# PSeitz/veloci

Measured on AMD Instinct MI355X. Metric: queries/sec, 3-term AND on 100M-doc index (p50 latency and HBM fraction alongside), higher is better.
Workload: dtype u32 doc ids + f16->f32 scores

## Files before the change

### veloci_amd/csrc/capi.cpp

```cpp
#include <chrono>
#include <thread>
#include <cstdio>
#include <cstdlib>
#include <cstring>

#include "../../include/veloci_amd.h"
#include <functional>
#include <future>

#include <dlfcn.h>
#include <unistd.h>

#include "engine.hpp"
#include "text.hpp"

using namespace vq;
using vqreq::Request;
using vqreq::VelociError;

namespace {
thread_local std::string g_err;

int fail(int code, const std::string& msg) {
    g_err = msg;
// ... 1547 lines not shown
    ~vq_shard_step() {
        pbs.clear();
        if (idx && idx->comm && idx->comm->unmerged == this) idx->comm->unmerged = nullptr;
        if (counted && idx && idx->comm) {
            idx->comm->live -= 1;
            idx->comm->busy[parity] = false;
        }
    }
};
namespace {
void comm_fail(ShardComm& c, const std::string& why) {
    if (!c.failed.empty()) return;
    c.failed = why;
    if (c.nccl) {
        try {
            if (rccl_api().CommAbort) (void)rccl_api().CommAbort(static_cast<ncclComm_t>(c.nccl));
            c.nccl = nullptr;
        } catch (...) {
        }
    }
}
void bounded_wait(const Index& idx, ShardComm& c, hipEvent_t ev) {
    static const long limit_ms = [] {
        const char* e = std::getenv("VQ_STEP_TIMEOUT_MS");
        return e ? std::atol(e) : 120000L;
    }();
    const auto t0 = std::chrono::steady_clock::now();
    for (uint64_t spins = 0;; ++spins) {
        const hipError_t q = hipEventQuery(ev);
        if (q == hipSuccess) return;
        if (q != hipErrorNotReady) {
            comm_fail(c, std::string("the step's stream reported ") + hipGetErrorString(q));
            throw VelociError(VQ_ERR_DEVICE, "sharded step: " + c.failed);
        }
        if (spins < 2000) continue;
        if ((spins & 63u) == 0) {
            if (c.nccl && rccl_api().CommGetAsyncError) {
                int aerr = 0;
                if (rccl_api().CommGetAsyncError(static_cast<ncclComm_t>(c.nccl), &aerr) == 0 && aerr != 0) {
                    comm_fail(c, std::string("RCCL reported ") + (rccl_api().GetErrorString ? rccl_api().GetErrorString(aerr) : "an error") + " while the step was in flight (a rank is gone)");
                    throw VelociError(VQ_ERR_DEVICE, "sharded step: " + c.failed);
                }
            }
            const long waited = long(std::chrono::duration_cast<std::chrono::milliseconds>(std::chrono::steady_clock::now() - t0).count());
            if (limit_ms > 0 && waited > limit_ms) {
                comm_fail(c, "a step did not complete within " + std::to_string(limit_ms) + " ms (VQ_STEP_TIMEOUT_MS): a rank did not join its exchange");
                throw VelociError(VQ_ERR_DEVICE, "sharded step: " + c.failed);
            }
        }
        std::this_thread::sleep_for(std::chrono::microseconds(20));
    }
    (void)idx;
}
void step_queue_merge(vq_shard_step& step) {
    if (step.merge_queued) return;
    step.merge_queued = true;
    const Index& idx = *step.idx;
    ShardComm& c = *idx.comm;
    if (c.unmerged == &step) c.unmerged = nullptr;
    if (step.used) VQ_HIP(hipStreamWaitEvent(idx.fin_stream, c.ev_xchg[step.parity], 0));
    const uint8_t* gathered = static_cast<const uint8_t*>(c.gathered[step.parity].p);
    for (size_t k = 0; k < step.pbs.size(); ++k)
        finish_launch(idx, *step.pbs[k], step.used && step.pbs[k]->nq_dev ? gathered + step.arena_off[k] : nullptr, uint32_t(c.nranks));
    VQ_HIP(hipEventRecord(c.ev_fin[step.parity], idx.fin_stream));
}
}

int vq_shard_step_begin(const vq_index* index, const vq_request* const* requests, size_t n, vq_shard_step** out) {
    return guard([&] {
        if (!index || !out || (n && !requests)) throw VelociError(VQ_ERR_INVALID_ARGUMENT, "vq_shard_step_begin: null argument");
        *out = nullptr;
        const Index& idx = *index->idx;
        if (!idx.comm) {
            auto local = std::make_unique<ShardComm>();
            comm_setup(const_cast<Index&>(idx), std::move(local));
        }
        ShardComm& c = *idx.comm;
        if (!c.failed.empty()) throw VelociError(VQ_ERR_DEVICE, "vq_shard_step_begin: the communicator is down (" + c.failed + "): make it again (vq_comm_init / vq_comm_init_custom) on every rank");
        const bool exchange = c.nccl != nullptr || c.allgather != nullptr;
        static const bool timing = std::getenv("VQ_TIMING") != nullptr;
        const auto tb0 = std::chrono::steady_clock::now();
        VQ_HIP(hipSetDevice(idx.device));
        const std::vector<const Request*> reqs = request_pointers(requests, n);
        if (c.unmerged) {
            vq_shard_step& prev = *static_cast<vq_shard_step*>(c.unmerged);
            step_queue_merge(prev);
            VQ_HIP(hipStreamWaitEvent(idx.stream, c.ev_fin[prev.parity], 0));
        }
        const auto tb1 = std::chrono::steady_clock::now();
        if (c.live >= 2) throw VelociError(VQ_ERR_INVALID_ARGUMENT, "vq_shard_step_begin: two steps are in flight already (end one first)");
        auto step = std::make_unique<vq_shard_step>();
        step->idx = &idx;
        step->counted = true;
        c.live += 1;
        step->n = n;
        step->parity = c.busy[0] ? 1 : 0;
        if (c.busy[step->parity]) {
            step->counted = false;
            c.live -= 1;
            throw VelociError(VQ_ERR_INVALID_ARGUMENT, "vq_shard_step_begin: both step slots are held (end a step first)");
        }
        c.busy[step->parity] = true;
        auto tb2 = tb1;
        try {
        const size_t chunks_env = [] {
            const char* e = std::getenv("VQ_SHARD_CHUNKS");
            return size_t(e ? std::min(2, std::max(1, std::atoi(e))) : 0);
        }();
        const size_t nchunks = chunks_env && n >= 512 ? chunks_env : 1;
        for (size_t k = 0; k < nchunks; ++k) {
            const size_t b = n * k / nchunks, e = n * (k + 1) / nchunks;
            step->first.push_back(b);
            step->pbs.push_back(run_partial(idx, reqs.data() + b, e - b, step->parity * 2 + int(k)));
        }
        tb2 = std::chrono::steady_clock::now();
        size_t off = 0;
        for (auto& pb : step->pbs) {
            step->arena_off.push_back(off);
            if (exchange && pb->nq_dev) off += (size_t(pb->layout.off_hist) * size_t(c.nranks) + 255) / 256 * 256;
        }
        step->used = off;
        if (off) {
            VQ_HIP(hipEventRecord(c.ev_scan[step->parity], idx.stream));
            VQ_HIP(hipStreamWaitEvent(c.stream, c.ev_scan[step->parity], 0));
            c.gathered[step->parity].ensure(off);
            uint8_t* gathered = c.gathered[step->parity].as<uint8_t>();
            for (size_t k = 0; k < step->pbs.size(); ++k) {
                PartialBatch& pb = *step->pbs[k];
                if (!pb.nq_dev) continue;
                const size_t bytes = size_t(pb.layout.off_hist);
                if (c.nccl) nccl_check(rccl_api().AllGather(pb.d_partial, gathered + step->arena_off[k], bytes, kNcclUint8, static_cast<ncclComm_t>(c.nccl), c.stream), "ncclAllGather");
                else if (c.allgather(c.ctx, pb.d_partial, gathered + step->arena_off[k], bytes, c.stream) != 0) throw VelociError(VQ_ERR_DEVICE, "sharded step: the caller's all-gather failed");
                if (pb.layout.total_hist) {
                    void* h = pb.d_partial + pb.layout.off_hist;
                    if (c.nccl) nccl_check(rccl_api().AllReduce(h, h, size_t(pb.layout.total_hist), kNcclUint32, kNcclSum, static_cast<ncclComm_t>(c.nccl), c.stream), "ncclAllReduce");
                    else if (!c.allreduce_u32 || c.allreduce_u32(c.ctx, h, size_t(pb.layout.total_hist), c.stream) != 0)
                        throw VelociError(VQ_ERR_DEVICE, "sharded step: the caller's all-reduce failed");
                }
            }
            VQ_HIP(hipEventRecord(c.ev_xchg[step->parity], c.stream));
        }
        } catch (const std::exception& ex) {
            if (exchange && c.nranks > 1) comm_fail(c, std::string("a step failed on rank ") + std::to_string(c.rank) + ": " + ex.what());
            throw;
        }
        c.unmerged = step.get();
        *out = step.release();
        if (timing) {
            const auto tb3 = std::chrono::steady_clock::now();
            auto ms = [](auto a, auto b) { return std::chrono::duration<double, std::milli>(b - a).count(); };
            std::fprintf(stderr, "[vq timing] shard step begin %.3f ms (queue the previous merge %.3f, compile + scans %.3f, exchange calls %.3f)\n", ms(tb0, tb3), ms(tb0, tb1), ms(tb1, tb2), ms(tb2, tb3));
        }
    });
}

int vq_shard_step_end(vq_shard_step* step_raw, size_t stride, uint64_t* num_hits, uint32_t* counts, uint32_t* ids, float* scores, int* status) {
    std::unique_ptr<vq_shard_step> step(step_raw);
    return guard([&] {
        if (!step || (step->n && (!num_hits || !counts || !ids || !scores))) throw VelociError(VQ_ERR_INVALID_ARGUMENT, "vq_shard_step_end: null argument");
        const Index& idx = *step->idx;
        ShardComm& c = *idx.comm;
        VQ_HIP(hipSetDevice(idx.device));
        static const bool timing = std::getenv("VQ_TIMING") != nullptr;
        const auto te0 = std::chrono::steady_clock::now();
        if (!c.failed.empty()) throw VelociError(VQ_ERR_DEVICE, "vq_shard_step_end: the communicator is down (" + c.failed + ")");
        step_queue_merge(*step);
// ... 86 lines not shown
```

### veloci_amd/csrc/engine.hpp

```cpp
#pragma once
#include <hip/hip_runtime.h>

#include <atomic>
#include <cmath>
#include <chrono>
#include <cstdint>
#include <cstdlib>
#include <map>
#include <limits>
#include <memory>
#include <thread>
#include <functional>
#include <condition_variable>
#include <mutex>
#include <string>
#include <unordered_map>
#include <vector>

#include "device_types.hpp"
#include "kernels.hpp"
#include "request.hpp"
#include "hostpool.hpp"
#include "regex_dfa.hpp"

// ... 456 lines not shown
    void* unmerged = nullptr;
    int live = 0;
    DevBuf gathered[2];
    DevBuf red;
    bool busy[2] = {false, false};
    std::string failed;
    std::mutex mu;
    ~ShardComm();
};

struct Index {
    int device = 0;
    int (*allreduce_fn)(void*, uint64_t*, size_t) = nullptr;
    void* allreduce_ctx = nullptr;
    bool sharded() const { return doc_lo != 0 || doc_hi != num_anchors; }
    bool can_sum_over_shards() const { return !sharded() || allreduce_fn != nullptr; }
    void sum_over_shards(std::vector<uint64_t>& v) const {
        if (!sharded() || v.empty()) return;
        if (!allreduce_fn || allreduce_fn(allreduce_ctx, v.data(), v.size()) != 0) throw vqreq::VelociError(vqreq::ERR_DEVICE, "all-reduce over the shards failed");
    }
    struct HighlightField {
        std::once_flag once;
        bool ok = false;
        uint32_t num_texts = 0;
        const KVStore* t2t = nullptr;
        const KVStore* tokens = nullptr;
        const uint32_t* d_vals = nullptr;
        DevBuf own_vals;
    };
    mutable std::mutex highlight_mu;
    mutable std::map<std::string, std::unique_ptr<HighlightField>> highlight_fields;
    mutable std::atomic<uint64_t> highlight_device_parts{0}, highlight_snippets_built{0};
    mutable std::atomic<uint64_t> suggest_topn_probes{0}, suggest_records_back{0};
    mutable std::atomic<uint64_t> or_reruns{0};
    mutable std::unique_ptr<HostPool> pool;
    mutable std::mutex pool_mu;
    uint64_t uid = 0;
    uint32_t num_anchors = 0, doc_lo = 0, doc_hi = 0;
    uint32_t bitmap_base = 0;
    uint64_t bitmap_words = 0;
    std::map<std::string, Dictionary> dict;
    std::map<std::string, PostingStore> postings;
    std::map<std::string, KVStore> kv;
    std::map<std::string, PhraseStore> phrase;
    std::map<std::string, BoostColumn> boost;
    std::map<std::string, ColumnMeta> columns;
    uint64_t device_bytes = 0;
    mutable std::mutex composed_mu;
    mutable std::map<std::string, std::unique_ptr<KVStore>> composed_facets;
    const KVStore& composed_facet(const std::vector<std::string>& steps) const;
    hipStream_t own_stream = nullptr, own_fin_stream = nullptr;
    hipStream_t pre_stream = nullptr;
    hipStream_t stream = nullptr;
    hipStream_t fin_stream = nullptr;
    mutable std::mutex profile_mutex;
    mutable Profile profile;
    mutable Workspace ws[kWorkspaces];
    mutable std::atomic<uint32_t> next_ws{0};
    mutable DevBuf arena;
    static constexpr size_t kArenaBytes = 64ull << 20;
    mutable std::unique_ptr<ShardComm> comm;
    ~Index();
    bool is_anchor_identity(const std::string& textindex_path) const;
};

std::unique_ptr<Index> build_index(const IndexBuilder& b, int device);

struct DocSet {
    uint64_t index_uid = 0;
    uint32_t num_anchors = 0, doc_lo = 0, doc_hi = 0;
    uint64_t len = 0;
    uint32_t local_len = 0;
    uint64_t bitmap_words = 0, rank_entries = 0, tile_entries = 0;
    DevBuf docs, bitmap, rank_dir, tile_dir;
    uint64_t device_bytes = 0;
    float ms_mark = -1.0f, ms_count_scan = -1.0f, ms_expand = -1.0f;
    int route = -1;
    int device = 0;
    hipStream_t stream = nullptr;
};
using DocSetMarkFn = std::function<void(hipStream_t st, uint32_t* scratch, uint64_t scratch_words, unsigned long long* meta)>;
std::shared_ptr<DocSet> docset_from_marks(const Index& idx, hipStream_t st, uint64_t n, const DocSetMarkFn& mark);
inline uint64_t docset_scratch_words(const Index& idx) { return ((uint64_t(idx.num_anchors) + 511u) / 512u) * 16u; }
std::shared_ptr<const DocSet> make_docset(const Index& idx, const uint32_t* ids, uint64_t n, bool on_device);
std::shared_ptr<const DocSet> make_docset_from_program(const Index& idx, hipStream_t st, const DList* lists, uint32_t n_lists, const DOp* fops, uint32_t n_fops,
                                                       uint32_t stack_depth);
enum { SETOP_AND = 0, SETOP_OR = 1, SETOP_MINUS = 2, SETOP_NOT = 3 };
std::shared_ptr<const DocSet> combine_docsets(const Index& idx, int op, const std::vector<std::shared_ptr<const DocSet>>& sets);
uint64_t copy_docset_ids(const DocSet& ds, uint32_t* out, uint64_t cap, bool on_device);

struct HList {
    const uint32_t* d_docs = nullptr;
    const uint16_t* d_scores = nullptr;
    uint32_t len = 0;
    uint32_t flags = 0;
    float term_score = 0.f;
    uint16_t max_raw = 0x7C00;
    uint16_t pivot_raw = 0x7C00;
    float max_value = std::numeric_limits<float>::infinity();
    uint64_t global_len = 0;
    const uint32_t* d_bitmap = nullptr;
    const uint32_t* d_rank_dir = nullptr;
    const uint32_t* d_tile_dir = nullptr;
    const uint32_t* d_cov32 = nullptr;
    const uint16_t* d_arr16 = nullptr;
    const uint32_t* d_gdir = nullptr;
// ... 114 lines not shown
    uint32_t n_spans = 0, tile_words = 0;
    struct Node {
        uint32_t id;
        uint64_t hits, hits_in_filter;
    };
    std::vector<Node> nodes;
};
std::vector<NodeCounts> debug_node_counts(const Index& idx, const vqreq::Request* const* reqs, size_t n, bool summed);
struct Result;
void complete_explain_requests(const Index& idx, std::vector<std::unique_ptr<Result>>& results, std::vector<int>& status, std::vector<std::string>& errors);
void complete_why_found_requests(const Index& idx, std::vector<std::unique_ptr<Result>>& results, std::vector<int>& status, std::vector<std::string>& errors);
bool request_wants_explain(const vqreq::Request& req);
std::string explain_records_json(const ExplainRecs& records);
void complete_deep_requests(const Index& idx, const vqreq::Request* const* reqs, size_t n, std::vector<std::unique_ptr<Result>>& results,
                            std::vector<int>& status, std::vector<std::string>& errors);

struct ResultFacet {
    std::string field;
    std::vector<std::pair<std::string, uint64_t>> entries;
};
struct Result {
    uint64_t num_hits = 0;
    uint64_t execution_time_ns = 0;
    std::vector<uint32_t> ids;
    std::vector<float> scores;
    std::vector<ResultFacet> facets;
    bool has_facets = false;
    std::map<std::string, std::vector<std::string>> why_found_terms;
    std::shared_ptr<const ExplainPlan> explain_plan;
    std::shared_ptr<const WhyFoundPlan> why_found_plan;
    std::map<uint32_t, std::map<std::string, std::vector<std::string>>> why_found_info;
    bool has_explain = false;
    std::vector<std::pair<bool, ExplainRecs>> explain;
    bool deep = false;
    bool rerun_exact = false;
    mutable std::string json;
};

struct PartialBatch {
    const Index* index = nullptr;
    Workspace* ws = nullptr;
    std::unique_lock<std::mutex> lock;
    bool pinned_ws = false;
    std::vector<CompiledQuery> queries;
    std::vector<uint32_t> slot;
    std::vector<uint8_t> qclass;
    std::vector<FacetJob> facet_jobs;
    uint32_t nq_dev = 0;
    PartialLayout layout{};
    const uint8_t* d_blobs = nullptr;
    const uint32_t* d_blob_off = nullptr;
    const FacetJob* d_facet_jobs = nullptr;
    uint8_t* d_partial = nullptr;
    uint32_t total_spans = 0;
    uint32_t n_facet_jobs = 0;
    uint32_t total_facet_out = 0;
    bool profiled = false;
    bool launched = false, finished = false;
    bool merge_launched = false;
    std::chrono::steady_clock::time_point t0;
    void release_workspace();
    std::vector<const vqreq::Request*> reqs;
    ~PartialBatch();
};

std::unique_ptr<PartialBatch> run_partial(const Index& idx, const vqreq::Request* const* reqs, size_t n, int slot = -1, int64_t arena_offset = -1);
void finish_batch(const Index& idx, PartialBatch& pb, const void* gathered_device, uint32_t num_shards, std::vector<std::unique_ptr<Result>>& out,
                  std::vector<int>& status, std::vector<std::string>& errors, size_t shard_stride = 0);
void finish_launch(const Index& idx, PartialBatch& pb, const void* gathered_device, uint32_t num_shards, size_t shard_stride = 0);

}
```

### veloci_amd/csrc/exec.cpp

```cpp
#include <algorithm>
#include <cstdio>
#include <cstdlib>
#include <cstring>
#include <thread>

#include "engine.hpp"
#include "staging.hpp"

#include "text.hpp"

namespace vq {

using namespace vqreq;

void DevBuf::ensure(size_t n) {
    if (n <= bytes) return;
    size_t want = std::max(n, bytes + bytes / 2);
    alloc(want);
}
PinnedBuf::~PinnedBuf() {
    if (p) (void)hipHostFree(p);
}
void PinnedBuf::ensure(size_t n) {
    if (n <= bytes) return;
// ... 612 lines not shown
        t.qmap = reinterpret_cast<uint32_t*>(hup + up_qmap) + at;
        t.d_span_base = reinterpret_cast<const uint32_t*>(dup + up_span) + at;
        t.d_qmap = reinterpret_cast<const uint32_t*>(dup + up_qmap) + at;
        at += t.n + 1;
        t.n = 0;
    }
    qi = 0;
    for (const CompiledQuery& cq : pb.queries) {
        if (cq.status != 0) continue;
        const uint32_t ti = table_of(cq);
        ScanTable& t = P.tabs[ti];
        t.span_base[t.n] = t.spans;
        t.qmap[t.n++] = qi;
        t.spans += cq.n_spans;
        const uint32_t n_scatter = cq.simple_n - uint32_t(__builtin_popcount(sf_bitmap_mask(cq.simple_flags)));
        switch (cq.kclass) {
            case K_SCAN_WIDE:
                P.leaves_wide = std::max<uint32_t>(P.leaves_wide, cq.wide.n_leaves);
                P.scatter_wide = std::max<uint32_t>(P.scatter_wide, cq.wide.n_leaves - uint32_t(__builtin_popcount(cq.wide.bitmap_mask)));
                break;
            case K_SCAN_RICH:
                P.facets_rich = P.facets_rich || !cq.facets.empty();
                P.scatter_rich = std::max<uint32_t>(P.scatter_rich, n_scatter + cq.simple2.n_side);
                break;
            case K_SCAN_UNION: P.union_has_or = P.union_has_or || cq.simple_n > 1; break;
            case K_SCAN_PROBE: {
                ScanPlan::ProbeParams& pp = P.probe[ti - T_PROBE];
                pp.na_seen |= 1u << uint32_t(__builtin_popcount(sf_array_mask(cq.simple_flags)));
                pp.arr_slot = std::max(pp.arr_slot, cq.probe_arr_gran * 4u);
                P.any_probe = true;
                break;
            }
            case K_SCAN_AND: P.scatter_and = std::max(P.scatter_and, n_scatter); break;
            case K_SCAN_SIMPLE: P.scatter_simple = std::max(P.scatter_simple, n_scatter); break;
            default: break;
        }
        pb.qclass.push_back(uint8_t(cq.kclass));
        P.cls_layout[cq.kclass] += cq.layout_bytes;
        P.cls_algo[cq.kclass] += cq.algorithmic_bytes;
        P.cls_q[cq.kclass] += 1;
        ++qi;
    }
    for (ScanTable& t : P.tabs) t.span_base[t.n] = t.spans;
    if (!pb.facet_jobs.empty()) std::memcpy(hup + up_jobs, pb.facet_jobs.data(), pb.facet_jobs.size() * sizeof(FacetJob));
    pb.d_blobs = dup;
    pb.d_blob_off = reinterpret_cast<const uint32_t*>(dup + up_blob_off);
    pb.d_facet_jobs = reinterpret_cast<const FacetJob*>(dup + up_jobs);
    return P;
}

static void launch_scans(const Index& idx, PartialBatch& pb, const BatchLayout& L, const ScanPlan& P, int64_t arena_offset) {
    Workspace& ws = *pb.ws;
    const PartialLayout& lay = pb.layout;
    hipStream_t st = idx.stream;
    VQ_HIP(hipMemcpyAsync(ws.d_up.as<uint8_t>(), ws.h_up.as<uint8_t>(), P.up_bytes, hipMemcpyHostToDevice, st));
    ws.d_span_keys.ensure(size_t(L.total_span_keys) * 8 + 16);
    if (arena_offset >= 0) {
        if (size_t(arena_offset) % 256 || size_t(arena_offset) + lay.bytes > Index::kArenaBytes)
            throw VelociError(ERR_UNSUPPORTED, "partial arena: the step's partials do not fit (" + std::to_string(size_t(arena_offset) + lay.bytes) + " bytes)");
        idx.arena.ensure(Index::kArenaBytes);
        pb.d_partial = idx.arena.as<uint8_t>() + arena_offset;
    } else {
        ws.d_partial.ensure(lay.bytes);
        pb.d_partial = ws.d_partial.as<uint8_t>();
    }
    VQ_HIP(hipMemsetAsync(pb.d_partial, 0, lay.bytes, st));

    uint32_t max_top_k = 1;
    uint32_t desc_cap = 0;
    bool facets_generic = false;
    static const bool no_facet_cache = std::getenv("VQ_NO_FACET_CACHE") != nullptr;
    for (const CompiledQuery& cq : pb.queries) {
        if (cq.status != 0) continue;
        max_top_k = std::max(max_top_k, cq.top_k);
        desc_cap = std::max(desc_cap, uint32_t(cq.desc_bytes));
        if (cq.kclass == K_TILE_SCAN && !cq.facets.empty()) facets_generic = !no_facet_cache;
    }
    desc_cap = uint32_t(align_up(desc_cap, 16));
    if (facets_generic) desc_cap += 2 * 1024 * 4;
    static const uint32_t cand_min = [] {
        const char* e = std::getenv("VQ_CAND_CAP");
        return uint32_t(e ? std::max(32, std::atoi(e)) : 32);
    }();
    uint32_t cand_cap = cand_min;
    while (cand_cap < 2 * max_top_k) cand_cap <<= 1;
    const uint32_t list_table = (std::max<uint32_t>(L.max_lists, 2) + 1u) & ~1u;
    static const bool tile_queue = std::getenv("VQ_NO_QUEUE") == nullptr;
    size_t lds_bytes = 0;
    for (const CompiledQuery& cq : pb.queries)
        if (cq.status == 0 && cq.kclass == K_TILE_SCAN)
            lds_bytes = std::max(lds_bytes, tile_scan_lds_bytes(uint32_t(cq.lists.size()) + cq.n_temps, uint32_t(cq.lists.size()), cq.tile_words, L.stack_depth, cand_cap, desc_cap,
                                                                tile_queue && !cq.simple_n, list_table));
    if (lds_bytes > 160 * 1024) throw VelociError(ERR_UNSUPPORTED, "LDS tile larger than 160 KiB");

    auto hits_ptr = reinterpret_cast<unsigned long long*>(pb.d_partial + lay.off_hits);
    auto hist_ptr = reinterpret_cast<uint32_t*>(pb.d_partial + lay.off_hist);
    auto keys_ptr = ws.d_span_keys.as<unsigned long long>();
    auto scan = [&](uint32_t table, int k, auto&& launch) {
        if (const ScanTable& t = P.tabs[table]; t.spans) {
            LaunchTimer lt(pb.profiled, ws, st, k, P.cls_layout[k], P.cls_algo[k], P.cls_q[k]);
            launch(t);
        }
        VQ_HIP(hipGetLastError());
    };
    scan(T_LEAF_F32, K_SCAN_LEAF_F32, [&](const ScanTable& t) { launch_scan_leaf_f32(st, t.spans, pb.d_blobs, pb.d_blob_off, t.d_span_base, t.d_qmap, t.n, cand_cap, keys_ptr, hits_ptr, hist_ptr); });
    scan(T_RICH, K_SCAN_RICH, [&](const ScanTable& t) { launch_scan_simple(st, true, P.scatter_rich, t.spans, pb.d_blobs, pb.d_blob_off, t.d_span_base, t.d_qmap, t.n, cand_cap, keys_ptr, hits_ptr, hist_ptr, P.facets_rich); });
    if (P.any_probe) {
        LaunchTimer lt(pb.profiled, ws, st, K_SCAN_PROBE, P.cls_layout[K_SCAN_PROBE], P.cls_algo[K_SCAN_PROBE], P.cls_q[K_SCAN_PROBE]);
        static const bool trace = std::getenv("VQ_PROBE_TRACE") != nullptr;
        for (uint32_t c = 0; c < kProbeShapes; ++c)
            if (const ScanTable& t = P.tabs[T_PROBE + c]; t.spans && trace)
                std::fprintf(stderr, "probe launch: shape %u, %u queries, %u spans, array slot %u words (fullest tile: %u granules), NA seen 0x%x\n", c, t.n, t.spans,
                             P.probe[c].arr_slot, P.probe[c].arr_slot / 4, P.probe[c].na_seen);
        for (uint32_t c = 0; c < kProbeShapes; ++c)
            if (const ScanTable& t = P.tabs[T_PROBE + c]; t.spans)
                launch_scan_probe_shape(st, c, P.probe[c].na_seen, P.probe[c].arr_slot, t.spans, pb.d_blobs, pb.d_blob_off, t.d_span_base, t.d_qmap, t.n, cand_cap, keys_ptr, hits_ptr);
    }
    VQ_HIP(hipGetLastError());
    scan(T_AND, K_SCAN_AND, [&](const ScanTable& t) { launch_scan_simple(st, false, P.scatter_and, t.spans, pb.d_blobs, pb.d_blob_off, t.d_span_base, t.d_qmap, t.n, cand_cap, keys_ptr, hits_ptr, hist_ptr); });
    scan(T_SIMPLE, K_SCAN_SIMPLE, [&](const ScanTable& t) { launch_scan_simple(st, false, P.scatter_simple, t.spans, pb.d_blobs, pb.d_blob_off, t.d_span_base, t.d_qmap, t.n, cand_cap, keys_ptr, hits_ptr, hist_ptr); });
    scan(T_UNION, K_SCAN_UNION, [&](const ScanTable& t) { launch_scan_union(st, P.union_has_or, t.spans, pb.d_blobs, pb.d_blob_off, t.d_span_base, t.d_qmap, t.n, cand_cap, keys_ptr, hits_ptr); });
    scan(T_WIDE, K_SCAN_WIDE, [&](const ScanTable& t) { launch_scan_wide(st, P.leaves_wide, P.scatter_wide, t.spans, pb.d_blobs, pb.d_blob_off, t.d_span_base, t.d_qmap, t.n, cand_cap, keys_ptr, hits_ptr); });
    scan(T_TILE, K_TILE_SCAN, [&](const ScanTable& t) { launch_tile_scan(st, t.spans, lds_bytes, pb.d_blobs, pb.d_blob_off, t.d_span_base, t.d_qmap, t.n, L.stack_depth, cand_cap, desc_cap, keys_ptr, hits_ptr, hist_ptr, tile_queue, list_table, facets_generic); });
    {
        LaunchTimer t(pb.profiled, ws, st, K_MERGE_SPANS, L.total_span_keys * 8 + L.total_keys * 8, L.total_span_keys * 8 + L.total_keys * 8, L.nq);
        launch_merge_spans(st, L.nq, pb.d_blobs, pb.d_blob_off, keys_ptr, reinterpret_cast<unsigned long long*>(pb.d_partial + lay.off_keys));
    }
    VQ_HIP(hipGetLastError());
    VQ_HIP(hipEventRecord(ws.ev_done, st));
    pb.launched = true;
}

static void report_timing(size_t n, double t_start, const CompileReport& c, double t_layout, double t_packed, const ScanTable* tabs) {
    if (!timing_enabled()) return;
    std::fprintf(stderr, "[vq timing] n=%zu compile %.3f ms (dictionary scans %.3f [%zu probes], pass 1 %.3f, unions %.3f [%zu jobs], pass 2 %.3f), range jobs %.3f [%zu], spans generic/simple/and/rich/union %u/%u/%u/%u/%u, pack+launch %.3f ms\n", n,
                 c.t_compiled - t_start, c.t_probes - t_start, c.probes, c.t_pass1 - c.t_probes, c.t_unions - c.t_pass1, c.unions, c.t_compiled - c.t_ranges,
                 c.t_ranges - c.t_unions, c.ranges, tabs[T_TILE].spans, tabs[T_SIMPLE].spans, tabs[T_AND].spans, tabs[T_RICH].spans, tabs[T_UNION].spans + tabs[T_LEAF_F32].spans, now_ms() - c.t_compiled);
    std::fprintf(stderr, "[vq timing] pack+launch: span sizing + layout %.3f, blobs + tables %.3f, upload + launches %.3f ms\n", t_layout - c.t_compiled, t_packed - t_layout, now_ms() - t_packed);
    uint64_t v[16];
    for (int k = 0; k < 16; ++k) v[k] = g_compile_ns[k].exchange(0);
    if (std::getenv("VQ_TIMING_SUB")) {
        std::fprintf(stderr, "[vq timing] inside 1:n resolve (thread-ms; 6 value-id gather, 7 sort, 8 pairs, 9 order check + layers):");
        for (int k = 6; k < 10; ++k) std::fprintf(stderr, " [%d] %.3f", k, v[k] * 1e-6);
        std::fprintf(stderr, "\n");
    }
    std::fprintf(stderr, "[vq timing] compile thread-ms: total %.3f = dictionary lookups %.3f + 1:n resolve %.3f + 1:n layers %.3f + leaf lists %.3f + rest %.3f; longest request %.3f\n", v[5] * 1e-6,
                 v[0] * 1e-6, v[1] * 1e-6, (v[2] - v[1]) * 1e-6, v[3] * 1e-6, (double(v[5]) - double(v[0]) - double(v[2]) - double(v[3])) * 1e-6, v[4] * 1e-6);
}

std::unique_ptr<PartialBatch> run_partial(const Index& idx, const vqreq::Request* const* reqs, size_t n, int slot, int64_t arena_offset) {
    const double t_start = now_ms();
    auto pb = std::make_unique<PartialBatch>();
    pb->index = &idx;
    pb->reqs.assign(reqs, reqs + n);
    pb->t0 = std::chrono::steady_clock::now();
    acquire_workspace(idx, *pb, slot);
    VQ_HIP(hipSetDevice(idx.device));
    Workspace& ws = *pb->ws;
    ws.timed.clear();
    ws.ev_used = 0;
    pb->profiled = idx.profile.enabled;

    const CompileReport compiled = compile_batch(idx, ws, *pb, reqs, n, idx.stream);
    size_spans(pb->queries);
    const BatchLayout layout = plan_layout(idx, *pb);
    const double t_layout = now_ms();
    const ScanPlan plan = pack_upload(idx, *pb, layout);
    if (layout.nq == 0) return pb;
    const double t_packed = now_ms();
    launch_scans(idx, *pb, layout, plan, arena_offset);
    report_timing(n, t_start, compiled, t_layout, t_packed, plan.tabs);
    return pb;
}

static void account_timed_launches(Profile& P, Workspace& ws) {
    P.batches += 1;
    for (const TimedLaunch& t : ws.timed) {
        float ms = 0.f;
        if (hipEventElapsedTime(&ms, ws.ev_pool[t.ev_begin], ws.ev_pool[t.ev_end]) != hipSuccess) continue;
        KernelProfile& k = P.k[t.kernel];
        k.ms += ms;
        k.launches += 1;
        k.layout_bytes += t.layout_bytes;
        k.algorithmic_bytes += t.algorithmic_bytes;
        k.queries += t.queries;
    }
    ws.timed.clear();
}

void debug_prepass(const Index& idx, const std::function<void(Workspace&, hipStream_t)>& body) {
    VQ_HIP(hipSetDevice(idx.device));
    Workspace& ws = idx.ws[idx.next_ws.fetch_add(1) % kWorkspaces];
    std::unique_lock<std::mutex> lock(ws.mu);
    ws.timed.clear();
    ws.ev_used = 0;
    const hipStream_t st = idx.pre_stream ? idx.pre_stream : idx.stream;
    body(ws, st);
    VQ_HIP(hipStreamSynchronize(st));
    if (idx.profile.enabled) {
        std::lock_guard<std::mutex> g(idx.profile_mutex);
        account_timed_launches(idx.profile, ws);
    }
}

static hipStream_t compile_without_scan(const Index& idx, Workspace& ws, PartialBatch& pb, const vqreq::Request* const* reqs, size_t n, BatchTables& tables) {
    pb.index = &idx;
    CompileReport rep;
    return compile_before_counts(idx, ws, pb, reqs, n, idx.stream, tables, rep);
}

std::vector<NodeCounts> debug_node_counts(const Index& idx, const vqreq::Request* const* reqs, size_t n, bool summed) {
    std::vector<NodeCounts> out(n);
    debug_prepass(idx, [&](Workspace& ws, hipStream_t) {
        PartialBatch pb;
        BatchTables tables;
        const hipStream_t pst = compile_without_scan(idx, ws, pb, reqs, n, tables);
// ... 763 lines not shown
        if (status[owner[k]] != 0) results[owner[k]].reset();
    }
}

PartialBatch::~PartialBatch() {
    if (ws && launched && !finished && ws->ev_done) (void)hipEventSynchronize(ws->ev_done);
    release_workspace();
}
void PartialBatch::release_workspace() {
    if (!lock.owns_lock()) return;
    if (ws && pinned_ws) {
        ws->pinned.store(false, std::memory_order_release);
        pinned_ws = false;
    }
    lock.unlock();
}

namespace {
struct DownLayout {
    size_t K, J, F, o_hits, o_n, o_ids, o_scores, o_fn, o_fv, o_fc, o_stat, bytes;
    explicit DownLayout(const PartialBatch& pb) {
        const uint32_t nq = pb.nq_dev;
        K = size_t(pb.layout.total_keys);
        J = pb.n_facet_jobs;
        F = pb.total_facet_out;
        o_hits = 0;
        o_n = align_up(o_hits + size_t(nq) * 8, 16);
        o_ids = align_up(o_n + size_t(nq) * 4, 16);
        o_scores = align_up(o_ids + K * 4, 16);
        o_fn = align_up(o_scores + K * 4, 16);
        o_fv = align_up(o_fn + J * 4, 16);
        o_fc = align_up(o_fv + F * 4, 16);
        o_stat = align_up(o_fc + F * 4, 16);
        bytes = align_up(o_stat + size_t(nq) * 8, 256);
    }
};
}

void finish_launch(const Index& idx, PartialBatch& pb, const void* gathered_device, uint32_t num_shards, size_t shard_stride) {
    if (pb.merge_launched) return;
    pb.merge_launched = true;
    Workspace& ws = *pb.ws;
    hipStream_t st = idx.fin_stream;
    const PartialLayout& lay = pb.layout;
    const uint32_t nq = pb.nq_dev;
    VQ_HIP(hipSetDevice(idx.device));
    const DownLayout D(pb);
    const size_t K = D.K, J = D.J;
    if (!nq) return;
    const uint8_t* gathered = gathered_device ? static_cast<const uint8_t*>(gathered_device) : pb.d_partial;
    if (!gathered_device) num_shards = 1;
    ws.d_down.ensure(D.bytes);
    ws.h_down.ensure(D.bytes);
    if (st != idx.stream) VQ_HIP(hipStreamWaitEvent(st, ws.ev_done, 0));
    uint8_t* dd = ws.d_down.as<uint8_t>();
    const bool prof = pb.profiled;
    {
        LaunchTimer t(prof, ws, st, K_FINALIZE, uint64_t(num_shards) * (K * 8 + nq * 8) + K * 8, uint64_t(num_shards) * (K * 8 + nq * 8) + K * 8, nq);
        launch_finalize(st, nq, pb.d_blobs, pb.d_blob_off, gathered, num_shards, shard_stride ? shard_stride : size_t(lay.off_hist), lay, reinterpret_cast<uint32_t*>(dd + D.o_ids),
                        reinterpret_cast<float*>(dd + D.o_scores), reinterpret_cast<uint32_t*>(dd + D.o_n), reinterpret_cast<unsigned long long*>(dd + D.o_hits));
    }
    VQ_HIP(hipGetLastError());
    if (J) {
        const uint32_t* hist = reinterpret_cast<const uint32_t*>(pb.d_partial + lay.off_hist);
        LaunchTimer t(prof, ws, st, K_FACET_SELECT, lay.total_hist * 4, lay.total_hist * 4, J);
        launch_facet_select(st, uint32_t(J), pb.d_facet_jobs, hist, reinterpret_cast<uint32_t*>(dd + D.o_fv), reinterpret_cast<uint32_t*>(dd + D.o_fc),
                            reinterpret_cast<uint32_t*>(dd + D.o_fn));
        VQ_HIP(hipGetLastError());
    }
    VQ_HIP(hipMemcpyAsync(ws.h_down.p, dd, D.o_stat, hipMemcpyDeviceToHost, st));
    if (prof)
        VQ_HIP(hipMemcpyAsync(ws.h_down.as<uint8_t>() + D.o_stat, pb.d_partial + lay.off_stats, size_t(nq) * 8, hipMemcpyDeviceToHost, st));
}

void finish_batch(const Index& idx, PartialBatch& pb, const void* gathered_device, uint32_t num_shards, std::vector<std::unique_ptr<Result>>& out,
                  std::vector<int>& status, std::vector<std::string>& errors, size_t shard_stride) {
    const size_t n = pb.queries.size();
    out.clear();
    out.resize(n);
    status.assign(n, 0);
    errors.assign(n, std::string());
    finish_launch(idx, pb, gathered_device, num_shards, shard_stride);
    Workspace& ws = *pb.ws;
    hipStream_t st = idx.fin_stream;
    const PartialLayout& lay = pb.layout;
    const uint32_t nq = pb.nq_dev;
    const DownLayout D(pb);
    const size_t o_hits = D.o_hits, o_n = D.o_n, o_ids = D.o_ids, o_scores = D.o_scores, o_fn = D.o_fn, o_fv = D.o_fv, o_fc = D.o_fc;
    if (nq) {
        const bool prof = pb.profiled;
        VQ_HIP(hipStreamSynchronize(st));
        const uint64_t* gathered_bytes = reinterpret_cast<const uint64_t*>(ws.h_down.as<uint8_t>() + D.o_stat);
        pb.finished = true;
        if (prof) {
            std::lock_guard<std::mutex> g(idx.profile_mutex);
            Profile& P = idx.profile;
            account_timed_launches(P, ws);
            for (uint32_t q = 0; q < nq && q < pb.qclass.size(); ++q) {
                P.k[pb.qclass[q]].layout_bytes += gathered_bytes[q];
                P.k[pb.qclass[q]].gathered_bytes += gathered_bytes[q];
            }
        }
    }
    const uint64_t ns = uint64_t(std::chrono::duration_cast<std::chrono::nanoseconds>(std::chrono::steady_clock::now() - pb.t0).count());
    const double t_synced = now_ms();

    const uint8_t* hd = ws.h_down.as<uint8_t>();
// ... 98 lines not shown
```

### veloci_amd/csrc/index.cpp

```cpp
#include <algorithm>
#include <atomic>
#include <chrono>
#include <cstring>
#include <exception>
#include <mutex>
#include <thread>
#include <sys/mman.h>

#include "engine.hpp"
#include "text.hpp"

namespace vq {

uint16_t score_class_pivot(const uint16_t* sc, uint32_t len, uint16_t max_raw) {
    if (len == 0 || max_raw >= 0x7C00u) return max_raw;
    std::vector<uint32_t> count(size_t(max_raw) + 1, 0u);
    for (uint32_t i = 0; i < len; ++i) ++count[sc[i]];
    const uint64_t need = (uint64_t(len) + kScoreClassDiv - 1) / kScoreClassDiv;
    uint64_t above = 0;
    for (uint32_t r = max_raw; r-- > 0;) {
        above += count[r + 1];
        if (above >= need && count[r]) return uint16_t(r);
    }
    return max_raw;
}

const char* const TOKENS_TO_TEXT_ID = ".tokens_to_text_id";
const char* const TO_ANCHOR_ID_SCORE = ".to_anchor_id_score";
const char* const PHRASE_PAIR_TO_ANCHOR = ".phrase_pair_to_anchor";
const char* const VALUE_ID_TO_PARENT = ".value_id_to_parent";
const char* const PARENT_TO_VALUE_ID = ".parent_to_value_id";
const char* const TEXT_ID_TO_ANCHOR = ".text_id_to_anchor";
const char* const ANCHOR_TO_TEXT_ID = ".anchor_to_text_id";
const char* const BOOST_VALID_TO_VALUE = ".boost_valid_to_value";
const char* const TOKEN_VALUES = ".token_values";
const char* const VALUE_ID_TO_ANCHOR = ".value_id_to_anchor";
const char* const TEXTINDEX = ".textindex";

static bool ends_with(const std::string& s, const char* suf) {
    size_t n = std::strlen(suf);
    return s.size() >= n && std::memcmp(s.data() + s.size() - n, suf, n) == 0;
}

void DevBuf::alloc(size_t n) {
    release();
    bytes = n;
    if (n == 0) return;
    VQ_HIP(hipMalloc(&p, n));
}
void DevBuf::release() {
    if (p) (void)hipFree(p);
    p = nullptr;
    bytes = 0;
}
void DevBuf::upload(const void* src, size_t n, hipStream_t st) {
    if (n == 0) return;
    if (st) VQ_HIP(hipMemcpyAsync(p, src, n, hipMemcpyHostToDevice, st));
    else VQ_HIP(hipMemcpy(p, src, n, hipMemcpyHostToDevice));
}

Index::~Index() {
    for (auto& w : ws) {
        for (auto e : w.ev_pool)
            if (e) (void)hipEventDestroy(e);
        if (w.ev_done) (void)hipEventDestroy(w.ev_done);
    }
    if (own_stream) (void)hipStreamDestroy(own_stream);
    if (own_fin_stream) (void)hipStreamDestroy(own_fin_stream);
    if (pre_stream) (void)hipStreamDestroy(pre_stream);
}

bool Index::is_anchor_identity(const std::string& textindex_path) const {
    std::string field = textindex_path;
    if (ends_with(field, TEXTINDEX)) field.resize(field.size() - std::strlen(TEXTINDEX));
    auto it = columns.find(field);
    return it != columns.end() && it->second.is_anchor_identity_column;
}

static uint16_t f32_to_f16_rne(float f) {
    uint32_t x;
    std::memcpy(&x, &f, 4);
    const uint32_t sign = (x >> 16) & 0x8000u;
    const uint32_t exp = (x >> 23) & 0xFFu;
    uint32_t man = x & 0x7FFFFFu;
    if (exp == 0xFF) return uint16_t(sign | 0x7C00u | (man ? (0x200u | (man >> 13)) : 0));
    const int32_t e = int32_t(exp) - 112;
    if (e >= 0x1F) return uint16_t(sign | 0x7C00u);
    if (e <= 0) {
        if (e < -10) return uint16_t(sign);
        man |= 0x800000u;
        const uint32_t shift = uint32_t(14 - e);
        uint32_t hm = man >> shift;
        const uint32_t rb = 1u << (shift - 1);
        if ((man & rb) && ((man & (rb - 1)) || (hm & 1))) hm++;
        return uint16_t(sign | hm);
    }
    uint32_t h = sign | (uint32_t(e) << 10) | (man >> 13);
    if ((man & 0x1000u) && ((man & 0xFFFu) || (h & 1))) h++;
    return uint16_t(h);
}

static void append_padded(std::vector<uint32_t>& dst, const uint32_t* b, const uint32_t* e) {
    dst.insert(dst.end(), b, e);
    while (dst.size() & 3u) dst.push_back(0xFFFFFFFFu);
}

static void shard_subrange(const uint32_t* b, const uint32_t* e, uint32_t lo, uint32_t hi, const uint32_t** ob, const uint32_t** oe) {
    *ob = std::lower_bound(b, e, lo);
    *oe = std::lower_bound(*ob, e, hi);
}

void* big_alloc(size_t bytes) {
    void* p = mmap(nullptr, bytes, PROT_READ | PROT_WRITE, MAP_PRIVATE | MAP_ANONYMOUS, -1, 0);
    if (p == MAP_FAILED) throw std::bad_alloc();
    (void)madvise(p, bytes, MADV_HUGEPAGE);
    return p;
}
void big_free(void* p, size_t bytes) noexcept { munmap(p, bytes); }

void parallel_for(size_t n, size_t threads, const std::function<void(size_t)>& fn) {
    threads = std::min(threads, n);
    if (threads <= 1) {
        for (size_t i = 0; i < n; ++i) fn(i);
        return;
    }
    std::atomic<size_t> next{0};
    std::mutex err_mu;
    std::exception_ptr err;
    auto body = [&] {
        for (size_t i; (i = next.fetch_add(1, std::memory_order_relaxed)) < n;) {
            try {
                fn(i);
            } catch (...) {
                std::lock_guard<std::mutex> g(err_mu);
                if (!err) err = std::current_exception();
                next.store(n, std::memory_order_relaxed);
            }
        }
    };
    std::vector<std::thread> workers;
    for (size_t k = 1; k < threads; ++k) workers.emplace_back(body);
    body();
    for (auto& w : workers) w.join();
    if (err) std::rethrow_exception(err);
}

std::unique_ptr<Index> build_index(const IndexBuilder& b, int device) {
    int ndev = 0;
    hipError_t de = hipGetDeviceCount(&ndev);
    if (de != hipSuccess || ndev <= 0)
        throw VelociError(vqreq::ERR_DEVICE, std::string("no HIP device available (hipGetDeviceCount: ") + hipGetErrorString(de) + ", count " +
                                                 std::to_string(ndev) + "): the veloci_amd query path needs an MI355X (no CPU fallback)");
    if (device < 0 || device >= ndev) throw VelociError(vqreq::ERR_INVALID_ARGUMENT, "device index out of range");
    VQ_HIP(hipSetDevice(device));

    auto idx = std::make_unique<Index>();
    idx->device = device;
    static std::atomic<uint64_t> next_uid{1};
    idx->uid = next_uid.fetch_add(1);
    idx->num_anchors = b.num_anchors;
    idx->doc_lo = b.doc_lo;
    idx->doc_hi = b.doc_hi;
    idx->columns = b.columns;
    VQ_HIP(hipStreamCreateWithFlags(&idx->own_stream, hipStreamNonBlocking));
    {
        int lo = 0, hi = 0;
        VQ_HIP(hipDeviceGetStreamPriorityRange(&lo, &hi));
        VQ_HIP(hipStreamCreateWithPriority(&idx->own_fin_stream, hipStreamNonBlocking, hi));
    }
    VQ_HIP(hipStreamCreateWithFlags(&idx->pre_stream, hipStreamNonBlocking));
    idx->stream = idx->own_stream;
    idx->fin_stream = idx->own_fin_stream;
    for (auto& w : idx->ws) {
        VQ_HIP(hipEventCreateWithFlags(&w.ev_done, hipEventDisableTiming));
    }
    const uint32_t lo = b.doc_lo, hi = b.doc_hi;
    idx->bitmap_base = lo & ~65535u;
    idx->bitmap_words = ((uint64_t(hi) - idx->bitmap_base + 65535u) / 65536u) * 2048u + 2048u;

    for (auto& [path, f] : b.fst) {
        Dictionary d;
        d.terms = f.terms;
        d.lower_map.reserve(d.terms.size());
        for (uint32_t i = 0; i < d.terms.size(); ++i) d.lower_map[vqtext::to_lower_utf8(d.terms[i])].push_back(i);
        {
            std::vector<uint32_t> off(d.terms.size() + 1, 0u);
            std::vector<uint32_t> raw, low;
            std::vector<uint64_t> seen(0x110000 / 64, 0ull);
            for (uint32_t i = 0; i < d.terms.size(); ++i) {
                d.max_term_bytes = std::max(d.max_term_bytes, d.terms[i].size());
                for (uint32_t cp : vqtext::decode_utf8(d.terms[i])) {
                    if (cp < 0x110000u) seen[cp >> 6] |= 1ull << (cp & 63u);
                    else d.alphabet.push_back(cp);
                    if (cp > 0xFFFFu) d.char_bytes = 4;
                    if (cp == 0x130u) d.low_exact = false;
                    raw.push_back(cp);
                    low.push_back(vqtext::lower_cp(cp));
                }
                off[i + 1] = uint32_t(raw.size());
            }
            auto image = [&](DevBuf& dst, const std::vector<uint32_t>& cps) {
                if (d.char_bytes == 4) {
                    dst.alloc(cps.size() * 4 + 16);
                    dst.upload(cps.data(), cps.size() * 4);
                } else {
                    const std::vector<uint16_t> narrow(cps.begin(), cps.end());
                    dst.alloc(narrow.size() * 2 + 16);
                    dst.upload(narrow.data(), narrow.size() * 2);
                }
            };
            d.d_off.alloc(off.size() * 4 + 16);
            d.d_off.upload(off.data(), off.size() * 4);
            image(d.d_raw, raw);
            image(d.d_low, low);
            idx->device_bytes += d.d_off.bytes + d.d_raw.bytes + d.d_low.bytes;
            for (uint32_t w = 0; w < seen.size(); ++w)
                for (uint64_t bits = seen[w]; bits; bits &= bits - 1) d.alphabet.push_back(w * 64u + uint32_t(__builtin_ctzll(bits)));
            std::sort(d.alphabet.begin(), d.alphabet.end());
            d.alphabet.erase(std::unique(d.alphabet.begin(), d.alphabet.end()), d.alphabet.end());
            d.alphabet_ascii = uint32_t(std::lower_bound(d.alphabet.begin(), d.alphabet.end(), 128u) - d.alphabet.begin());
            d.d_alpha.alloc((d.alphabet.size() - d.alphabet_ascii) * 4 + 16);
            d.d_alpha.upload(d.alphabet.data() + d.alphabet_ascii, (d.alphabet.size() - d.alphabet_ascii) * 4);
            idx->device_bytes += d.d_alpha.bytes;
// ... 411 lines not shown
```

Measured before the change: 179,600.

## Split step scan chunks across two streams and drop cross-step finalize wait

```diff
diff --git a/veloci_amd/csrc/capi.cpp b/veloci_amd/csrc/capi.cpp
--- a/veloci_amd/csrc/capi.cpp
+++ b/veloci_amd/csrc/capi.cpp
@@ -1623,6 +1623,20 @@
     }
     (void)idx;
 }
+hipStream_t step_scan_stream(const Index& idx, size_t k) {
+    static const bool one = [] {
+        const char* e = std::getenv("VQ_STEP_SCAN_STREAMS");
+        return e && std::atoi(e) == 1;
+    }();
+    return k && !one && idx.stream == idx.own_stream && idx.own_stream2 ? idx.own_stream2 : idx.stream;
+}
+bool step_waits_for_finalize(bool two_streams) {
+    static const int knob = [] {
+        const char* e = std::getenv("VQ_STEP_FIN_WAIT");
+        return e ? int(std::atoi(e) != 0) : -1;
+    }();
+    return knob >= 0 ? knob != 0 : !two_streams;
+}
 void step_queue_merge(vq_shard_step& step) {
     if (step.merge_queued) return;
     step.merge_queued = true;
@@ -1653,10 +1667,15 @@
         const auto tb0 = std::chrono::steady_clock::now();
         VQ_HIP(hipSetDevice(idx.device));
         const std::vector<const Request*> reqs = request_pointers(requests, n);
+        const hipStream_t second = exchange ? idx.stream : step_scan_stream(idx, 1);
+        const bool two_streams = second != idx.stream;
         if (c.unmerged) {
             vq_shard_step& prev = *static_cast<vq_shard_step*>(c.unmerged);
             step_queue_merge(prev);
-            VQ_HIP(hipStreamWaitEvent(idx.stream, c.ev_fin[prev.parity], 0));
+            if (step_waits_for_finalize(two_streams)) {
+                VQ_HIP(hipStreamWaitEvent(idx.stream, c.ev_fin[prev.parity], 0));
+                if (two_streams) VQ_HIP(hipStreamWaitEvent(second, c.ev_fin[prev.parity], 0));
+            }
         }
         const auto tb1 = std::chrono::steady_clock::now();
         if (c.live >= 2) throw VelociError(VQ_ERR_INVALID_ARGUMENT, "vq_shard_step_begin: two steps are in flight already (end one first)");
@@ -1682,7 +1701,7 @@
         for (size_t k = 0; k < nchunks; ++k) {
             const size_t b = n * k / nchunks, e = n * (k + 1) / nchunks;
             step->first.push_back(b);
-            step->pbs.push_back(run_partial(idx, reqs.data() + b, e - b, step->parity * 2 + int(k)));
+            step->pbs.push_back(run_partial(idx, reqs.data() + b, e - b, step->parity * 2 + int(k), -1, k ? second : idx.stream));
         }
         tb2 = std::chrono::steady_clock::now();
         size_t off = 0;
diff --git a/veloci_amd/csrc/engine.hpp b/veloci_amd/csrc/engine.hpp
--- a/veloci_amd/csrc/engine.hpp
+++ b/veloci_amd/csrc/engine.hpp
@@ -532,6 +532,7 @@
     hipStream_t own_stream = nullptr, own_fin_stream = nullptr;
     hipStream_t pre_stream = nullptr;
     hipStream_t stream = nullptr;
+    hipStream_t own_stream2 = nullptr;
     hipStream_t fin_stream = nullptr;
     mutable std::mutex profile_mutex;
     mutable Profile profile;
@@ -752,6 +753,7 @@
     const uint32_t* d_blob_off = nullptr;
     const FacetJob* d_facet_jobs = nullptr;
     uint8_t* d_partial = nullptr;
+    hipStream_t scan_stream = nullptr;
     uint32_t total_spans = 0;
     uint32_t n_facet_jobs = 0;
     uint32_t total_facet_out = 0;
@@ -764,7 +766,8 @@
     ~PartialBatch();
 };
 
-std::unique_ptr<PartialBatch> run_partial(const Index& idx, const vqreq::Request* const* reqs, size_t n, int slot = -1, int64_t arena_offset = -1);
+std::unique_ptr<PartialBatch> run_partial(const Index& idx, const vqreq::Request* const* reqs, size_t n, int slot = -1, int64_t arena_offset = -1,
+                                          hipStream_t scan_stream = nullptr);
 void finish_batch(const Index& idx, PartialBatch& pb, const void* gathered_device, uint32_t num_shards, std::vector<std::unique_ptr<Result>>& out,
                   std::vector<int>& status, std::vector<std::string>& errors, size_t shard_stride = 0);
 void finish_launch(const Index& idx, PartialBatch& pb, const void* gathered_device, uint32_t num_shards, size_t shard_stride = 0);
diff --git a/veloci_amd/csrc/exec.cpp b/veloci_amd/csrc/exec.cpp
--- a/veloci_amd/csrc/exec.cpp
+++ b/veloci_amd/csrc/exec.cpp
@@ -688,7 +688,7 @@
 static void launch_scans(const Index& idx, PartialBatch& pb, const BatchLayout& L, const ScanPlan& P, int64_t arena_offset) {
     Workspace& ws = *pb.ws;
     const PartialLayout& lay = pb.layout;
-    hipStream_t st = idx.stream;
+    hipStream_t st = pb.scan_stream;
     VQ_HIP(hipMemcpyAsync(ws.d_up.as<uint8_t>(), ws.h_up.as<uint8_t>(), P.up_bytes, hipMemcpyHostToDevice, st));
     ws.d_span_keys.ensure(size_t(L.total_span_keys) * 8 + 16);
     if (arena_offset >= 0) {
@@ -784,12 +784,13 @@
                  v[0] * 1e-6, v[1] * 1e-6, (v[2] - v[1]) * 1e-6, v[3] * 1e-6, (double(v[5]) - double(v[0]) - double(v[2]) - double(v[3])) * 1e-6, v[4] * 1e-6);
 }
 
-std::unique_ptr<PartialBatch> run_partial(const Index& idx, const vqreq::Request* const* reqs, size_t n, int slot, int64_t arena_offset) {
+std::unique_ptr<PartialBatch> run_partial(const Index& idx, const vqreq::Request* const* reqs, size_t n, int slot, int64_t arena_offset, hipStream_t scan_stream) {
     const double t_start = now_ms();
     auto pb = std::make_unique<PartialBatch>();
     pb->index = &idx;
     pb->reqs.assign(reqs, reqs + n);
     pb->t0 = std::chrono::steady_clock::now();
+    pb->scan_stream = scan_stream ? scan_stream : idx.stream;
     acquire_workspace(idx, *pb, slot);
     VQ_HIP(hipSetDevice(idx.device));
     Workspace& ws = *pb->ws;
@@ -797,7 +798,7 @@
     ws.ev_used = 0;
     pb->profiled = idx.profile.enabled;
 
-    const CompileReport compiled = compile_batch(idx, ws, *pb, reqs, n, idx.stream);
+    const CompileReport compiled = compile_batch(idx, ws, *pb, reqs, n, pb->scan_stream);
     size_spans(pb->queries);
     const BatchLayout layout = plan_layout(idx, *pb);
     const double t_layout = now_ms();
@@ -1667,7 +1668,7 @@
     if (!gathered_device) num_shards = 1;
     ws.d_down.ensure(D.bytes);
     ws.h_down.ensure(D.bytes);
-    if (st != idx.stream) VQ_HIP(hipStreamWaitEvent(st, ws.ev_done, 0));
+    if (st != pb.scan_stream) VQ_HIP(hipStreamWaitEvent(st, ws.ev_done, 0));
     uint8_t* dd = ws.d_down.as<uint8_t>();
     const bool prof = pb.profiled;
     {
diff --git a/veloci_amd/csrc/index.cpp b/veloci_amd/csrc/index.cpp
--- a/veloci_amd/csrc/index.cpp
+++ b/veloci_amd/csrc/index.cpp
@@ -68,6 +68,7 @@
     if (own_stream) (void)hipStreamDestroy(own_stream);
     if (own_fin_stream) (void)hipStreamDestroy(own_fin_stream);
     if (pre_stream) (void)hipStreamDestroy(pre_stream);
+    if (own_stream2) (void)hipStreamDestroy(own_stream2);
 }
 
 bool Index::is_anchor_identity(const std::string& textindex_path) const {
@@ -169,6 +170,7 @@
         VQ_HIP(hipStreamCreateWithPriority(&idx->own_fin_stream, hipStreamNonBlocking, hi));
     }
     VQ_HIP(hipStreamCreateWithFlags(&idx->pre_stream, hipStreamNonBlocking));
+    VQ_HIP(hipStreamCreateWithFlags(&idx->own_stream2, hipStreamNonBlocking));
     idx->stream = idx->own_stream;
     idx->fin_stream = idx->own_fin_stream;
     for (auto& w : idx->ws) {
```

New measurement: 190,800 (median of 6 runs). 6.3% higher.
